# safijari/yag-slam

Hardware: AMD Instinct MI355X
Metric: pose hypotheses/sec (higher is better)
Workload: dtype u8

## Files before the change

### include/yagmatch.h

```cpp
#ifndef YAGMATCH_H
#define YAGMATCH_H

#include <stdint.h>

#ifdef __cplusplus
extern "C" {
#endif

#define YM_VERSION 1

enum {
    YM_OK = 0,
    YM_ERR_INVALID = -1,
    YM_ERR_NO_DEVICE = -2,
    YM_ERR_HIP = -3,
    YM_ERR_UNSUPPORTED = -4,
    YM_ERR_RANGE = -5,
    YM_ERR_BUSY = -6
};

enum { YM_SEM_KARTO = 0, YM_SEM_YAGPY = 1 };

typedef struct ym_config {
    double angle_variance_penalty;
// ... 215 lines not shown
int ym_graph_chi2(ym_graph *g, double *chi2);
int ym_graph_linearise(ym_graph *g, double *chi2, double *diag9 , double *grad3 );
int ym_graph_solve(ym_graph *g, int band , double lambda, double cg_tol, int max_cg_iters ,
                   double *delta3 , double *precond3 , int32_t *band_used,
                   int32_t *cg_iterations, double *residual, int32_t *flags);
typedef struct ym_opt_params { int32_t iters, exact, max_cg_iters, band ; double lambda0, cg_tol; } ym_opt_params;
typedef struct ym_opt_report { double chi2_initial, chi2_final, lambda_final; int32_t lm_steps, accepted, cg_iterations, band, status; } ym_opt_report;
int ym_graph_optimize(ym_graph *g, const ym_opt_params *p, ym_opt_report *out);

typedef struct ym_grid_info {
    int32_t width, height, pitch;
    int32_t origin_x, origin_y;
    int32_t storage_w, storage_h;
    int32_t roi_x, roi_y, roi_w, roi_h;
    double offset_x, offset_y;
} ym_grid_info;
int ym_debug_grid_info(ym_matcher *m, int item, ym_grid_info *info);
int ym_debug_grid(ym_matcher *m, int item, uint8_t *out, int64_t out_bytes);
int ym_debug_sums(ym_matcher *m, int item, int pass, uint32_t *out, int64_t out_count);
int ym_debug_map_sums(ym_matcher *m, int item, int pass, uint32_t *out, int64_t out_count);
int ym_debug_query_local(ym_matcher *m, int item, double *out_xy, int32_t cap, int32_t *n);
int ym_debug_cells(ym_matcher *m, int item, int32_t *out, int64_t out_count, int32_t *max_n);

int ym_debug_option(ym_matcher *m, int option, int value);

#define YM_DEBUG_COUNTERS 8
int ym_debug_counters(ym_matcher *m, int64_t *out, int32_t count);

int ym_debug_live_bytes(int64_t *device_bytes, int64_t *pinned_bytes);

int ym_debug_stamps(ym_matcher *m, int enable, uint64_t *out, int32_t count);

int ym_profile_enable(ym_matcher *m, int on);
int ym_profile_read(ym_matcher *m, int which, double *ms_total, int64_t *launches, int reset);
int ym_cache_stats(const ym_matcher *m, int64_t *hits, int64_t *misses);

#ifdef __cplusplus
}
#endif
#endif
```

### yag_slam_amd/_capi.py

```python
import ctypes as C
import os
import subprocess

_HERE = os.path.dirname(os.path.abspath(__file__))
LIB_PATH = os.environ.get("YM_LIB_PATH") or os.path.join(_HERE, "libyagmatch.so")

YM_OK = 0
SEM = {"karto": 0, "yagpy": 1}

EXPORTS = (
    "ym_version", "ym_build_id", "ym_device_count", "ym_last_error", "ym_create", "ym_destroy", "ym_get_config",
    "ym_set_stream", "ym_synchronize", "ym_scan_create", "ym_scans_create", "ym_scans_destroy", "ym_scan_set_pose", "ym_scans_set_poses", "ym_scan_get_pose",
    "ym_scan_size", "ym_scan_structure_trusted", "ym_scan_destroy", "ym_match", "ym_match_scans", "ym_map_sequence", "ym_process_scan", "ym_sequence_stats", "ym_async_slots",
    "ym_match_scans_async", "ym_wait", "ym_match_batch", "ym_batch_create", "ym_batch_destroy", "ym_batch_size",
    "ym_match_pairs", "ym_pairs_create",
    "ym_batch_run_async", "ym_batch_wait", "ym_debug_grid_info",
    "ym_debug_grid", "ym_debug_sums", "ym_debug_query_local", "ym_debug_cells", "ym_debug_option", "ym_debug_stamps", "ym_debug_live_bytes",
    "ym_profile_enable",
    "ym_profile_read", "ym_cache_stats", "ym_debug_counters",
    "ym_coarse_dims", "ym_match_slice_begin", "ym_match_slice_finish",
    "ym_occupancy_create", "ym_occupancy_create_counted", "ym_occupancy_get_info", "ym_occupancy_read", "ym_occupancy_read_counts",
    "ym_occupancy_destroy", "ym_image_despeckle", "ym_occupancy_create_clean", "ym_occupancy_get_despeckle_stats",
    "ym_map_from_occupancy", "ym_map_from_grid", "ym_map_size", "ym_map_read", "ym_map_destroy", "ym_match_map",
    "ym_match_map_many", "ym_map_track", "ym_debug_map_sums",
    "ym_raymap_create", "ym_raymap_trace", "ym_raymap_trace_each", "ym_raymap_destroy",
    "ym_locator_create", "ym_locator_get_info", "ym_locator_read_level", "ym_locator_locate", "ym_locator_destroy",
    "ym_segments_create", "ym_segments_label_range", "ym_segments_stats", "ym_segments_boundaries", "ym_segments_pairs",
    "ym_segments_destroy", "ym_map_free_space", "ym_segments_from_map", "ym_segments_labels",
    "ym_graph_create", "ym_graph_destroy", "ym_graph_add_nodes", "ym_graph_add_constraints", "ym_graph_size", "ym_graph_set_poses",
    "ym_graph_get_poses", "ym_graph_chi2", "ym_graph_linearise", "ym_graph_solve", "ym_graph_optimize",
)


class YmError(RuntimeError):
    def __init__(self, code, msg):
        super().__init__("libyagmatch error %d: %s" % (code, msg))
        self.code = code


class YmConfig(C.Structure):
# ... 165 lines not shown
    L.ym_match.argtypes = [vp, C.POINTER(YmScanDesc), C.POINTER(YmScanDesc), C.c_int, C.c_int, C.c_int,
                           C.POINTER(YmResult)]
    L.ym_match_scans.argtypes = [vp, vp, C.POINTER(vp), C.c_int, C.c_int, C.c_int, C.POINTER(YmResult)]
    L.ym_async_slots.argtypes = [vp]
    L.ym_match_scans_async.argtypes = [vp, vp, C.POINTER(vp), C.c_int, C.c_int, C.c_int, C.c_int]
    L.ym_wait.argtypes = [vp, C.c_int, C.POINTER(YmResult)]
    L.ym_match_batch.argtypes = [vp, vp, C.POINTER(vp), ip, C.c_int, C.c_int, C.c_int, C.POINTER(YmResult),
                                 C.POINTER(YmResult), ip]
    L.ym_batch_create.restype = vp
    L.ym_batch_create.argtypes = [vp, vp, C.POINTER(vp), ip, C.c_int]
    L.ym_pairs_create.restype = vp
    L.ym_pairs_create.argtypes = [vp, C.POINTER(vp), C.POINTER(vp), ip, C.c_int]
    L.ym_match_pairs.argtypes = [vp, C.POINTER(vp), C.POINTER(vp), ip, C.c_int, C.c_int, C.c_int, C.POINTER(YmResult)]
    L.ym_batch_destroy.argtypes = [vp]
    L.ym_batch_destroy.restype = None
    L.ym_batch_size.argtypes = [vp]
    L.ym_batch_run_async.argtypes = [vp, vp, C.c_int, C.c_int, C.c_int, C.c_int64, vp]
    L.ym_batch_wait.argtypes = [vp, C.c_int, C.POINTER(YmResult), C.POINTER(YmResult), ip]
    L.ym_debug_grid_info.argtypes = [vp, C.c_int, C.POINTER(YmGridInfo)]
    L.ym_debug_grid.argtypes = [vp, C.c_int, C.POINTER(C.c_uint8), C.c_int64]
    L.ym_debug_sums.argtypes = [vp, C.c_int, C.c_int, C.POINTER(C.c_uint32), C.c_int64]
    L.ym_debug_query_local.argtypes = [vp, C.c_int, dp, C.c_int32, ip]
    L.ym_debug_cells.argtypes = [vp, C.c_int, ip, C.c_int64, ip]
    L.ym_debug_option.argtypes = [vp, C.c_int, C.c_int]
    L.ym_debug_stamps.argtypes = [vp, C.c_int, C.POINTER(C.c_uint64), C.c_int32]
    L.ym_debug_live_bytes.argtypes = [C.POINTER(C.c_int64), C.POINTER(C.c_int64)]
    L.ym_profile_enable.argtypes = [vp, C.c_int]
    L.ym_profile_read.argtypes = [vp, C.c_int, dp, C.POINTER(C.c_int64), C.c_int]
    L.ym_cache_stats.argtypes = [vp, C.POINTER(C.c_int64), C.POINTER(C.c_int64)]
    L.ym_debug_counters.argtypes = [vp, C.POINTER(C.c_int64), C.c_int32]
    L.ym_coarse_dims.argtypes = [vp, ip]
    L.ym_scan_structure_trusted.argtypes = [vp, C.c_int]
    L.ym_process_scan.argtypes = [vp, vp, C.POINTER(vp), C.c_int, dp, dp, C.c_int, C.c_int, C.POINTER(YmResult)]
    L.ym_sequence_stats.argtypes = [vp, C.POINTER(C.c_int64), C.POINTER(C.c_int64), C.POINTER(C.c_int64)]
    L.ym_map_sequence.argtypes = [vp, C.POINTER(vp), dp, C.c_int, C.c_int, C.c_int, C.c_int, C.c_int, C.c_int, C.POINTER(YmResult), ip]
    L.ym_match_slice_begin.argtypes = [vp, vp, C.POINTER(vp), C.c_int, C.c_int, C.c_int, C.c_int, C.c_int, vp, vp]
    L.ym_match_slice_finish.argtypes = [vp, C.POINTER(YmResult)]
    L.ym_occupancy_create.restype = vp
    L.ym_occupancy_create.argtypes = [C.POINTER(vp), C.c_int, C.c_double, C.c_double]
    L.ym_occupancy_create_counted.restype = vp
    L.ym_occupancy_create_counted.argtypes = [C.POINTER(vp), C.c_int, C.c_double, C.c_double]
    L.ym_occupancy_get_info.argtypes = [vp, C.POINTER(YmOccupancyInfo)]
    L.ym_occupancy_read.argtypes = [vp, C.POINTER(C.c_uint8), C.c_int64]
    L.ym_occupancy_read_counts.argtypes = [vp, C.POINTER(C.c_uint32), C.POINTER(C.c_uint32), C.c_int64]
    L.ym_occupancy_destroy.argtypes = [vp]
    L.ym_occupancy_destroy.restype = None
# ... 93 lines not shown
```

### yag_slam_amd/csrc/ym_abi_debug.hpp

```cpp
int ym_debug_grid_info(ym_matcher *m, int item, ym_grid_info *info) {
    if (!m || !info) return set_err(YM_ERR_INVALID, "null argument");
    if (!m->last_valid || item < 0 || item >= m->last_B) return set_err(YM_ERR_INVALID, "no such item in the last call");
    const YmGeom &g = m->last_geom;
    info->width = g.win_w; info->height = g.win_w; info->pitch = g.pitch;
    info->origin_x = g.win_origin; info->origin_y = g.win_origin;
    info->storage_w = g.storage_w; info->storage_h = g.storage_w;
    info->roi_x = g.border; info->roi_y = g.border; info->roi_w = g.roi_w; info->roi_h = g.roi_w;
    YmItemState s;
    DEV_GUARD(m->device);
    HIP_TRY(hipStreamSynchronize(m->stream));
    HIP_TRY(hipMemcpy(&s, m->states.p + item, sizeof s, hipMemcpyDeviceToHost));
    info->offset_x = s.off_x; info->offset_y = s.off_y;
    return YM_OK;
}

int ym_debug_grid(ym_matcher *m, int item, uint8_t *out, int64_t out_bytes) {
    if (!m || !out) return set_err(YM_ERR_INVALID, "null argument");
    if (!m->last_valid || item < 0 || item >= m->last_B) return set_err(YM_ERR_INVALID, "no such item in the last call");
    const int64_t need = (int64_t)m->last_geom.pitch * m->last_geom.win_w;
    if (out_bytes < need) return set_err(YM_ERR_INVALID, "grid buffer too small: need %lld bytes", (long long)need);
    DEV_GUARD(m->device);
    HIP_TRY(hipStreamSynchronize(m->stream));
    HIP_TRY(hipMemcpy(out, m->grid.p + (size_t)item * m->last_grid_stride, (size_t)need, hipMemcpyDeviceToHost));
    return YM_OK;
// ... 18 lines not shown
    if (!m || !out_xy || !n) return set_err(YM_ERR_INVALID, "null argument");
    if (!m->last_valid || item < 0 || item >= m->last_B) return set_err(YM_ERR_INVALID, "no such item in the last call");
    YmItemState s;
    DEV_GUARD(m->device);
    HIP_TRY(hipStreamSynchronize(m->stream));
    HIP_TRY(hipMemcpy(&s, m->states.p + item, sizeof s, hipMemcpyDeviceToHost));
    *n = s.nq;
    if (cap < s.nq) return set_err(YM_ERR_INVALID, "buffer too small: need %d points", s.nq);
    if (s.nq > 0)
        HIP_TRY(hipMemcpy(out_xy, s.ql, sizeof(double2) * s.nq, hipMemcpyDeviceToHost));
    return YM_OK;
}

int ym_debug_cells(ym_matcher *m, int item, int32_t *out, int64_t out_count, int32_t *max_n) {
    if (!m || !max_n) return set_err(YM_ERR_INVALID, "null argument");
    if (!m->last_valid || item < 0 || item >= m->last_B) return set_err(YM_ERR_INVALID, "no such item in the last call");
    *max_n = m->last_max_n;
    const size_t per = (size_t)m->last_max_base * m->last_max_n;
    if (!out) return YM_OK;
    if ((size_t)out_count < per * 2) return set_err(YM_ERR_INVALID, "buffer too small: need %zu ints", per * 2);
    DEV_GUARD(m->device);
    HIP_TRY(hipStreamSynchronize(m->stream));
    HIP_TRY(hipMemcpy(out, m->cells.p + (size_t)item * per, sizeof(int2) * per, hipMemcpyDeviceToHost));
    return YM_OK;
}

int ym_debug_option(ym_matcher *m, int option, int value) {
    if (m) { m->cache_gen++; m->list_key_valid = false; }
    if (!m) return set_err(YM_ERR_INVALID, "null matcher");
    if (option == 0) return set_err(YM_ERR_INVALID, "debug option 0 (an experimental correlate form) no longer exists");
    else if (option == 2) m->full_raster = value;
    else if (option == 3) m->corr_u = value;
    else if (option == 4) m->corr_pad_lds = value;
    else if (option == 5) m->corr_chunks = value;
    else if (option == 6) m->finish_form = value;
    else if (option == 9) m->corr_cw = value;
    else if (option == 10) m->select_global = value;
    else if (option == 41) m->select_split_max = value;
    else if (option == 11) m->finish_threads = value;
    else if (option == 12) m->keep_sums = value;
    else if (option == 13) m->corr_dedup = value;
    else if (option == 14) m->corr_region = value;
    else if (option == 15) m->corr_region_na = m->corr_region_nw = value;
    else if (option == 23) m->poll_completion = value != 0;
    else if (option == 24) m->use_scan_structure = value != 0;
    else if (option == 25) m->chain_margin = value;
// ... 148 lines not shown
```

### yag_slam_amd/csrc/ym_host_call.hpp

```cpp
int launch_call_body(ym_matcher *m, Slot &slot) {
    static const bool debug_host = getenv("YM_DEBUG_HOST") != nullptr;
    timespec t_[8];
    auto mark = [&](int i) { if (debug_host) clock_gettime(CLOCK_MONOTONIC, &t_[i]); };
    mark(7);
    DEV_GUARD(m->device);
    CallPlan P;
    int rc;
    mark(0);
    m->last_corr_form = -1;
    if ((rc = plan_sizes(m, slot, P))) return rc;
    mark(1);
    Call &pc = slot.call;
    const bool replay = pc.batch_uid != 0 && pc.plan_clean && pc.plan_gen == m->cache_gen && pc.pose_epoch == g_pose_epoch.load(std::memory_order_relaxed);
    if (!replay && (rc = plan_cache(m, slot, P))) return rc;
    mark(2);
    if ((rc = plan_jobs(m, slot, P, replay))) return rc;
    mark(3);
    if ((rc = plan_descriptor(m, slot, P, replay))) return rc;
    if (pc.batch_uid != 0 && !replay) {
        bool clean = !m->cache_off;
        for (const CallScan &cs : pc.scans) clean = clean && !cs.stale && !cs.qstale;
        pc.plan_clean = clean;
        pc.plan_gen = m->cache_gen;
    }
    mark(4);
    hipStream_t st = m->stream;
    hipEvent_t ev_call = nullptr;
    if ((rc = prof_begin(m, 2, &ev_call))) return rc;
    if ((rc = plan_raster(m, slot, P))) return rc;
    mark(5);

    timespec e_[8];
// ... 316 lines not shown
```

### yag_slam_amd/csrc/ym_host_enqueue.hpp

```cpp
void enqueue_prepare(ym_matcher *m, const CallPlan &P) {
    ym::PrepareArgs a;
    a.scans = P.d_scans; a.items = P.d_items; a.g = P.g; a.lat = P.lc; a.states = m->states.p; a.qlocal = m->qlocal.p;
    a.cells = m->cells.p; a.bbox = m->bbox.p; a.ctrig = m->ctrig.p; a.hypcell = m->hypcell.p; a.probs = P.probs;
    a.max_n = P.max_n; a.max_base = P.max_base; a.nt_stride = P.nt_stride; a.dim_stride = P.dim_stride; a.stamps = P.stamps;
    a.use_inline = P.inline_desc ? 1 : 0;
    a.pad0 = 0;
    std::memset(&a.inl, 0, sizeof a.inl);
    if (a.use_inline) {
        a.inl.item = P.hi[0];
        for (int i = 0; i < P.nscans; i++) a.inl.scans[i] = P.hs[i];
    }
    a.qnp = m->qnp.p; a.jobs = P.d_jobs; a.job_slot = P.d_job_slot;
    a.fault = nullptr; a.step = 0; a.pad1 = 0;
    for (int k = 0; k < 4; k++) a.cell_box[k] = P.cell_box[k];
    if (P.chain_step) { a.fault = m->seq_fault.p; a.step = P.chain_step; }
    a.tile_max_zero = P.use_tile_list ? m->tile_max.p : nullptr;
    const size_t lds = YM_PREP_LDS_BYTES(P.max_n);
    if (P.split_prepare) {
        if (P.n_jobs > 0) hipLaunchKernelGGL(ym::points_kernel, dim3(P.n_jobs), dim3(YM_POINTS_THREADS), lds, m->stream, a);
        hipLaunchKernelGGL(ym::cells_kernel, dim3(P.max_base + 1, P.B), dim3(256), 0, m->stream, a);
    } else {
        if (P.B == 1 && m->prepare_threads != 512)
            hipLaunchKernelGGL(ym::prepare_kernel<1024>, dim3(P.max_base + 2, P.B), dim3(1024), lds, m->stream, a);
        else
// ... 162 lines not shown
    if (P.rg2) { r.rg_h = P.rg2_h; r.rg_cls = YM_RG_PITCH * (P.rg2_h + 26); r.rg_zero = 4 * r.rg_cls; }
    r.pad2 = ((1 << 21) + r.rg_h - 1) / r.rg_h;
    r.rg_w = 0; r.rg_pitch = YM_RG_PITCH; r.nregions = P.rg_nregions; r.pad3 = 0;
    r.walk = m->rg_walk.p; r.nitems = P.B; r.rsplit = P.rg_rsplit; r.pad4 = 0;
    r.lnw = P.rg_lnw; r.lparts = P.rg_lparts; r.entries_pstride = P.rg_entries_pstride;
    r.gpx = std::max(1, std::min((2 * std::max(m->n_cus, 8) / 8) / std::max(1, P.rg_parts), (P.B + 7) / 8));
    return r;
}

int enqueue_region_lists(ym_matcher *m, const CallPlan &P, hipStream_t st) {
    const ym::RegionArgs r = region_args(m, P);
#ifdef YM_EXPERIMENTAL
    if (P.rg_lparts == 1 && P.rg_lnw == P.lc.nt && (P.rg_ws || P.rg2 || P.rg_item || P.rg_pool)) {
        const size_t bin_lds = YM_BIN_LDS_BYTES(P.rg_nbins, P.rg_entries_stride, P.rg_nregions * P.rg_parts);
        if (bin_lds > m->bin_lds_limit) {
            HIP_TRY(hipFuncSetAttribute(reinterpret_cast<const void *>(ym::bin_whole_kernel<false>), hipFuncAttributeMaxDynamicSharedMemorySize, (int)bin_lds));
            m->bin_lds_limit = bin_lds;
        }
        hipLaunchKernelGGL(ym::bin_whole_kernel<false>, dim3(P.n_qslots), dim3(YM_BIN_THREADS), bin_lds, st, r);
        if (P.rg_ws) hipLaunchKernelGGL(ym::region_walk_kernel, dim3(P.rg_parts, P.n_qslots), dim3(64), 0, st, r);
        return YM_OK;
    }
#endif
    const size_t bin_lds = YM_BINP_LDS_BYTES(P.rg_nbins, P.rg_entries_pstride, P.rg_nregions);
    if (bin_lds > m->binp_lds_limit) {
#define YM_BINP_ATTR(Y, M) HIP_TRY(hipFuncSetAttribute(reinterpret_cast<const void *>(ym::bin_kernel<Y, M>), hipFuncAttributeMaxDynamicSharedMemorySize, (int)bin_lds))
        YM_BINP_ATTR(false, 18); YM_BINP_ATTR(false, 32); YM_BINP_ATTR(false, 64); YM_BINP_ATTR(true, 18); YM_BINP_ATTR(true, 32); YM_BINP_ATTR(true, 64);
#undef YM_BINP_ATTR
        m->binp_lds_limit = bin_lds;
    }
    const int per_thread = (P.rg_lnw * P.max_n + YM_BINP_THREADS - 1) / YM_BINP_THREADS;
    const dim3 bgrid(P.rg_lparts, P.n_qslots);
#define YM_BINP_LAUNCH(Y, M) hipLaunchKernelGGL((ym::bin_kernel<Y, M>), bgrid, dim3(YM_BINP_THREADS), bin_lds, st, r)
    if (P.yag) { if (per_thread <= 18) YM_BINP_LAUNCH(true, 18); else if (per_thread <= 32) YM_BINP_LAUNCH(true, 32); else YM_BINP_LAUNCH(true, 64); }
    else { if (per_thread <= 18) YM_BINP_LAUNCH(false, 18); else if (per_thread <= 32) YM_BINP_LAUNCH(false, 32); else YM_BINP_LAUNCH(false, 64); }
#undef YM_BINP_LAUNCH
    return YM_OK;
}

int enqueue_region_lists_aside(ym_matcher *m, CallPlan &P) {
    if (!m->side_stream) {
        HIP_TRY(hipStreamCreateWithFlags(&m->side_stream, hipStreamNonBlocking));
        pool_register_stream(m->device, m->side_stream, true);
        HIP_TRY(hipEventCreateWithFlags(&m->ev_fork, hipEventDisableTiming));
        HIP_TRY(hipEventCreateWithFlags(&m->ev_join, hipEventDisableTiming));
    }
    HIP_TRY(hipEventRecord(m->ev_fork, m->stream));
    return YM_OK;
}
int enqueue_region_lists_joined(ym_matcher *m, CallPlan &P) {
    HIP_TRY(hipStreamWaitEvent(m->side_stream, m->ev_fork, 0));
    int rc = enqueue_region_lists(m, P, m->side_stream);
    if (rc) return rc;
    HIP_TRY(hipEventRecord(m->ev_join, m->side_stream));
    P.lists_on_side_stream = true;
    return YM_OK;
}

// ... 211 lines not shown
```

### yag_slam_amd/csrc/ym_host_matcher.hpp

```cpp
struct ym_map {
    int device;
    int width, height;
    DevBuf<double> d_cgrid;
    DevBuf<uint8_t> d_g8;
};

struct ym_occupancy {
    int device;
    ym_occupancy_info info;
    std::vector<uint8_t> image;
    std::vector<uint32_t> counts;
    bool cleaned = false;
    ym_despeckle_stats clean_stats{};
};

struct ym_batch {
    std::vector<const ym_scan *> queries;
    std::vector<int32_t> item_query;
    std::vector<const ym_scan *> scans;
    std::vector<int32_t> offsets;
    mutable std::vector<int> cache_hints;
    mutable std::vector<int> query_hints;
    uint64_t uid = 0;
};
// ... 126 lines not shown
    int corr_pad_lds = 0;
    int corr_cw = 0;
    int corr_dedup = 0;
    int corr_region = 0;
    int corr_region_na = 0;
    int corr_region_parts = 0;
    int corr_region_cap = 0;
    int corr_region_lds = 0;
    int raster_gx = 0;
    int raster_hits_per_tile = 0;
    int keep_sums = 0;
    int finish_threads = 0;
    int select_global = 0;
    int select_split_max = 8;
    DevBuf<double> tmp_ranges;
    PinnedBuf tmp_ranges_host;
    Slot slots[kAsyncSlots + 1];
    YmGeom last_geom;
    YmLattice last_lat[2];
    int last_B = 0, last_max_n = 0, last_max_base = 0, last_nt_stride = 0, last_dim_stride = 0;
    size_t last_grid_stride = 0, last_sums_stride[2] = {0, 0};
    size_t sums_pass_offset[2] = {0, 0};
    bool last_valid = false;
    bool profiling = false;
    ProfEvents prof[3];
};
```

### yag_slam_amd/csrc/ym_k_region.hpp

```cpp
#pragma once

namespace ym {

#ifndef YM_RG_PROF
#define YM_RG_PROF 0
#endif
#if YM_RG_PROF
#if YM_RG_PROF == 2
#define YM_RG_PH(i) do { if ((i) == 7 || (i) == 8 || (i) == 1 || (i) == 2 || (i) == 5) { const uint32_t t_ = (uint32_t)__builtin_amdgcn_s_memtime(); \
    if ((i) != 5) ph[(i) == 7 ? 0 : (i) == 8 ? 1 : (i) == 1 ? 2 : 3] += t_ - pt; pt = t_; } } while (0)
#else
#define YM_RG_PH(i) do { const uint32_t t_ = (uint32_t)__builtin_amdgcn_s_memtime(); if ((i) >= 2 && (i) <= 5) ph[(i) - 2] += t_ - pt; pt = t_; } while (0)
#endif
#else
#define YM_RG_PH(i) do { } while (0)
#endif

#ifndef YM_RG_ABLATE
#define YM_RG_ABLATE 0
#endif
#ifndef YM_RG_PRIO
#define YM_RG_PRIO 0
#endif
#define YM_RG_W 64
// ... 79 lines not shown
        const unsigned rx = xc / (unsigned)a.rg_w, ry = yc / (unsigned)a.rg_h;
        if ((int)rx >= a.nrx || (int)ry >= a.nry) return false;
        region = (int)((ry * (unsigned)a.nrx + rx) * 4u + cls);
        bin = region * a.lat.nt + k;
        er = yc - ry * (unsigned)a.rg_h;
        ex = xc - rx * (unsigned)a.rg_w;
        entry = er * (unsigned)a.rg_pitch + ex;
        return true;
    }
#endif
    if (yc >= 4096u) return false;
    const unsigned rx = xc / (unsigned)YM_RG_W, ry = __umul24(yc, (unsigned)a.pad2) >> 21;
    if ((int)rx >= a.nrx || (int)ry >= a.nry) return false;
    region = (int)(__umul24(ry, (unsigned)a.nrx) + rx);
    bin = (int)__umul24((unsigned)region, (unsigned)(bin_nw < 0 ? a.lat.nt : bin_nw)) + k;
    er = yc - __umul24(ry, (unsigned)a.rg_h);
    ex = xc - rx * YM_RG_W;
    entry = __umul24(cls, (unsigned)a.rg_cls) + __umul24(er, (unsigned)YM_RG_PITCH) + ex;
    return true;
}

#define YM_BINP_THREADS 512
#define YM_BINP_LDS_BYTES(nbins, entries, nboxes) ((size_t)(YM_BINP_THREADS / 64 + 16 + YM_RG_MAX_BINS / 32 + 1) * 4 + (size_t)(nbins) * 8 + ((size_t)(entries) * 2 + 15) / 16 * 16 + (size_t)(nboxes) * 16)
template <bool YAG, int MAXP>
__global__ __launch_bounds__(YM_BINP_THREADS, MAXP <= 18 ? 4 : 2) void bin_kernel(RegionArgs a) {
    constexpr int NT = YM_BINP_THREADS;
    extern __shared__ __attribute__((aligned(16))) unsigned char bin_smem[];
    int *wave_tot = reinterpret_cast<int *>(bin_smem);
    int *angle_tot = wave_tot + NT / 64;
    unsigned *region_bits = reinterpret_cast<unsigned *>(angle_tot + 16);
    int *regions_used = reinterpret_cast<int *>(region_bits + YM_RG_MAX_BINS / 32);
    unsigned (*cnt)[2] = reinterpret_cast<unsigned (*)[2]>(regions_used + 1);
    unsigned short *ent = reinterpret_cast<unsigned short *>(cnt + a.nbins);
    const int nboxes = a.nregions;
    unsigned (*box)[4] = reinterpret_cast<unsigned (*)[4]>(bin_smem + ((reinterpret_cast<unsigned char *>(ent + a.entries_pstride) - bin_smem) + 15) / 16 * 16);
    const int part = blockIdx.x, qs = blockIdx.y, b = a.qrep[qs], tid = threadIdx.x, lane = tid & 63;
    const YmItemState &st = a.states[b];
    const int nw = a.lnw, k_lo = part * nw, nk = min(a.lat.nt, k_lo + nw) - k_lo;
    const int nq = st.nq;
    const int total = nq * nk;
    const int32_t *cx = a.hypcell + (size_t)b * 2 * a.dim_stride;
    const int cx0 = cx[0], cy0 = cx[a.dim_stride];
    const double off_x = st.off_x, off_y = st.off_y;
    const double2 *ql = reinterpret_cast<const double2 *>(st.ql);
    const double2 *trig = a.ctrig + (size_t)b * a.nt_stride + k_lo;
    int32_t *starts = a.starts + (size_t)qs * a.starts_stride + (size_t)part * (a.nbins + 1);
    int32_t *flag = a.starts + (size_t)qs * a.starts_stride + (size_t)a.lparts * (a.nbins + 1) + part;
    const int pos0 = part * (int)a.entries_pstride;
    double2 *qls = reinterpret_cast<double2 *>(bin_smem + ((reinterpret_cast<unsigned char *>(ent) - bin_smem) + 15) / 16 * 16);
    const bool ql_in_lds = (size_t)(nq + nk) * sizeof(double2) + 16 <= (size_t)a.entries_pstride * 2;
    double2 *trigs = qls + nq;
    if (ql_in_lds) {
        for (int i = tid; i < nq; i += NT) qls[i] = ql[i];
        if (tid < nk) trigs[tid] = trig[tid];
    }
    for (int i = tid; i < a.nbins * 2; i += NT) (&cnt[0][0])[i] = 0u;
    if (tid < 16) angle_tot[tid] = 0;
    if (tid < YM_RG_MAX_BINS / 32) region_bits[tid] = 0u;
    if (tid == 0) *regions_used = 0;
    for (int i = tid; i < nboxes; i += NT) { box[i][0] = 255u; box[i][1] = 0u; box[i][2] = 255u; box[i][3] = 0u; }
    __syncthreads();
    unsigned key[MAXP];
    unsigned rank_hi[(MAXP + 3) / 4];
#pragma unroll
    for (int q = 0; q < (MAXP + 3) / 4; q++) rank_hi[q] = 0u;
    const int per_thread = (total + NT - 1) / NT;
    const int p0 = tid * per_thread;
    int k = p0 / max(nq, 1), i = p0 - k * nq;
    int cur = -1;
    unsigned r0 = 255u, r1 = 0u, x0 = 255u, x1 = 0u;
    auto send_box = [&]() {
        if (cur >= 0) {
            unsigned *bx = box[cur];
            atomicMin(&bx[0], r0); atomicMax(&bx[1], r1); atomicMin(&bx[2], x0); atomicMax(&bx[3], x1);
        }
    };
    bool overflow = per_thread > MAXP;
    auto pass1 = [&](auto point_of, auto trig_of) {
#pragma unroll
        for (int q = 0; q < MAXP; q++) {
            const int pp = p0 + q;
            key[q] = 0xffffffffu;
            if (q < per_thread && pp < total) {
                const double2 cs = trig_of(k);
                const double2 pt = point_of(i);
                int bin, region; unsigned e, er, ex;
                const int2 lc = YAG ? lookup_cell_sem(a.g, pt, cs.x, cs.y, off_x, off_y, st.ylat[0], st.ylat[1]) : lookup_cell(pt, cs.x, cs.y, off_x, off_y, a.g.scale);
                if (region_entry(a, lc, cx0, cy0, k, bin, e, region, er, ex, nw)) {
                    const unsigned rank = (atomicAdd(&cnt[bin][(e >> 1) & 1u], 1u << (16 * (e & 1u))) >> (16 * (e & 1u))) & 0xffffu;
                    key[q] = (rank & 7u) << 29 | (unsigned)bin << 16 | e;
                    rank_hi[q >> 2] |= ((rank >> 3) & 0xffu) << (8 * (q & 3));
                    if (region != cur) { send_box(); cur = region; r0 = r1 = er; x0 = x1 = ex; }
                    else { r0 = min(r0, er); r1 = max(r1, er); x0 = min(x0, ex); x1 = max(x1, ex); }
                }
            }
            if (++i >= nq) { i = 0; k++; }
        }
    };
    if (ql_in_lds) pass1([&](int i_) { return qls[i_]; }, [&](int k_) { return trigs[k_]; });
    else pass1([&](int i_) { return ql[i_]; }, [&](int k_) { return trig[k_]; });
    send_box();
    __syncthreads();
    {
        uint32_t *rb = a.rbox + (size_t)qs * a.rbox_stride;
        for (int r = tid; r < nboxes; r += NT) rb[(size_t)r * a.lparts + part] = box[r][0] | box[r][1] << 8 | box[r][2] << 16 | box[r][3] << 24;
    }
    const int per = (a.nbins + NT - 1) / NT;
    const int first = tid * per;
    int padded_total;
    {
        int local = 0;
        for (int j = 0; j < per; j++)
            if (first + j < a.nbins) {
                const unsigned c01 = cnt[first + j][0], c23 = cnt[first + j][1];
                const int c[4] = {(int)(c01 & 0xffffu), (int)(c01 >> 16), (int)(c23 & 0xffffu), (int)(c23 >> 16)};
                const int padded = (((c[0] + 1) & ~1) + ((c[1] + 1) & ~1) + ((c[2] + 1) & ~1) + ((c[3] + 1) & ~1) + 3) & ~3;
                local += padded;
                if (padded) {
                    atomicAdd(&angle_tot[(first + j) % nw], padded);
                    const int R = (first + j) / nw;
                    atomicOr(&region_bits[R >> 5], 1u << (R & 31));
                }
            }
// ... 26 lines not shown
                unsigned fill[4];
                for (int r = 0; r < 4; r++) {
                    fill[r] = (unsigned)pos;
                    if (fits && (c[r] & 1)) ent[pos + c[r]] = (unsigned short)(a.rg_zero + r);
                    pos += (c[r] + 1) & ~1;
                }
                if (fits && ((pos - run) & 3)) { ent[pos] = (unsigned short)a.rg_zero; ent[pos + 1] = (unsigned short)a.rg_zero; }
                pos = run + ((pos - run + 3) & ~3);
                cnt[first + j][0] = fill[0] | fill[1] << 16;
                cnt[first + j][1] = fill[2] | fill[3] << 16;
                run = pos;
            }
        if (tid == 0) {
            starts[a.nbins] = pos0 + all;
            *flag = fits ? all : -1;
            if (a.stamps && qs == 0 && part == 0) a.stamps[26] = (unsigned long long)all;
        }
        if (!fits) return;
    }
    __syncthreads();
#pragma unroll
    for (int q = 0; q < MAXP; q++) {
        if (key[q] == 0xffffffffu) continue;
        const unsigned bin = (key[q] >> 16) & 0x1fffu, e = key[q] & 0xffffu;
        const unsigned rank = key[q] >> 29 | ((rank_hi[q >> 2] >> (8 * (q & 3))) & 0xffu) << 3;
        const unsigned f = cnt[bin][(e >> 1) & 1u];
        ent[((e & 1u) ? f >> 16 : f & 0xffffu) + rank] = (unsigned short)e;
    }
    __syncthreads();
    uint32_t *out = reinterpret_cast<uint32_t *>(a.entries + (size_t)qs * a.entries_stride + pos0);
    const uint32_t *src = reinterpret_cast<const uint32_t *>(ent);
    for (int i2 = tid; i2 < (padded_total + 1) / 2; i2 += NT) out[i2] = src[i2];
}

typedef unsigned int rg_u32x2 __attribute__((ext_vector_type(2)));
__device__ __forceinline__ void rg_perm_pair(const rg_u32x2 &pa, const rg_u32x2 &qa, const rg_u32x2 &pb, const rg_u32x2 &qb, uint32_t rr,
                                             uint32_t (&e)[4], uint32_t (&o)[4]) {
    const uint32_t s0 = pa.x + pb.x, s1 = pa.y + pb.y, s2 = qa.x + qb.x, s3 = qa.y + qb.y;
    const uint32_t selE = rr * 0x00010001u + 0x0c020c00u, selO = selE + 0x00010001u;
    e[0] = __builtin_amdgcn_perm(s1, s0, selE); o[0] = __builtin_amdgcn_perm(s1, s0, selO);
    e[1] = __builtin_amdgcn_perm(s2, s1, selE); o[1] = __builtin_amdgcn_perm(s2, s1, selO);
    e[2] = __builtin_amdgcn_perm(s3, s2, selE); o[2] = __builtin_amdgcn_perm(s3, s2, selO);
    e[3] = __builtin_amdgcn_perm(0u, s3, selE);
    o[3] = 0u;
}
__device__ __forceinline__ void rg_gather4(uint32_t (&acc)[8], uint32_t lane_off, uint2 ee ) {
    const uint32_t ad0 = lane_off + (ee.x & 0xffffu), ad1 = lane_off + (ee.x >> 16), ad2 = lane_off + (ee.y & 0xffffu), ad3 = lane_off + (ee.y >> 16);
#if YM_RG_ABLATE & 1
    acc[0] += ad0 ^ ad1 ^ ad2 ^ ad3;
    return;
#endif
    rg_u32x2 p0, q0, p1, q1, p2, q2, p3, q3;
    asm volatile("ds_read2_b32 %0, %8 offset1:1\n\tds_read2_b32 %1, %8 offset0:2 offset1:3\n\t"
                 "ds_read2_b32 %2, %9 offset1:1\n\tds_read2_b32 %3, %9 offset0:2 offset1:3\n\t"
                 "ds_read2_b32 %4, %10 offset1:1\n\tds_read2_b32 %5, %10 offset0:2 offset1:3\n\t"
                 "ds_read2_b32 %6, %11 offset1:1\n\tds_read2_b32 %7, %11 offset0:2 offset1:3\n\t"
// ... 327 lines not shown
```

### yag_slam_amd/scan_matching.py

```python
import ctypes as C
import os
import struct
from collections import namedtuple

import numpy as np

from . import _capi
from .config import default_config, default_config_loop, make_config
from .models import LocalizedRangeScan
from .transform import Transform

ScanMatcherResult = namedtuple('ScanMatcherResult', ['response', 'covariance', 'best_pose', 'meta'])


def _pose_of(scan):
    p = scan.corrected_pose
    return float(p.x), float(p.y), float(p.euler[-1])


def _desc_of(scan, keep):
    d = _capi.YmScanDesc()
    r = np.ascontiguousarray(scan.ranges, dtype=np.float64)
    keep.append(r)
    d.ranges = r.ctypes.data_as(C.POINTER(C.c_double))
# ... 474 lines not shown
        _capi.check(self._lib.ym_debug_sums(self._m, item, pass_, buf.ctypes.data_as(C.POINTER(C.c_uint32)), buf.size))
        return buf

    def debug_map_sums(self, pass_=0, item=0, dims=None):
        nx, ny, nt = dims
        buf = np.zeros((nt, ny, nx), dtype=np.uint32)
        _capi.check(self._lib.ym_debug_map_sums(self._m, int(item), int(pass_), buf.ctypes.data_as(C.POINTER(C.c_uint32)), buf.size))
        return buf

    def debug_query_local(self, item=0, cap=8192):
        buf = np.zeros((cap, 2))
        n = C.c_int32()
        _capi.check(self._lib.ym_debug_query_local(self._m, item, buf.ctypes.data_as(C.POINTER(C.c_double)), cap,
                                                   C.byref(n)))
        return buf[:n.value].copy()

    def debug_cells(self, item=0, cap=1 << 16):
        buf = np.zeros((cap, 2), dtype=np.int32)
        max_n = C.c_int32()
        _capi.check(self._lib.ym_debug_cells(self._m, item, buf.ctypes.data_as(C.POINTER(C.c_int32)), buf.size,
                                             C.byref(max_n)))
        return buf.reshape(-1, 2), max_n.value

    def debug_option(self, option, value):
        _capi.check(self._lib.ym_debug_option(self._m, int(option), int(value)))

    def debug_stamps(self, enable=True):
        buf = (C.c_uint64 * 32)()
        _capi.check(self._lib.ym_debug_stamps(self._m, int(bool(enable)), buf, 32))
        return list(buf)

    def cache_stats(self):
        h, ms = C.c_int64(0), C.c_int64(0)
        _capi.check(self._lib.ym_cache_stats(self._m, C.byref(h), C.byref(ms)))
        return int(h.value), int(ms.value)

    def debug_counters(self):
        buf = (C.c_int64 * 8)()
        _capi.check(self._lib.ym_debug_counters(self._m, buf, 8))
        return dict(yag_fast_items=int(buf[0]), yag_fallback_items=int(buf[1]), yag_pairs_checked=int(buf[2]),
                    yag_pairs_failed=int(buf[3]), list_cache_hits=int(buf[4]), map_kernel_items=int(buf[6]), map_fallback_items=int(buf[7]),
                    last_correlate={-1: None, 0: "correlate_kernel", 1: "correlate_region_kernel", 2: "gather_kernel"}[int(buf[5])])

    def profile(self, on=True):
        _capi.check(self._lib.ym_profile_enable(self._m, int(bool(on))))

# ... 223 lines not shown
```

Before: 13.45 billion.

## Restructure bin kernel: angle-major thread mapping, LDS/memory variants, packed ranks

The region bin kernel now gives each thread a fixed angle and a contiguous run of query points, so trig is loaded once per thread and the per-point div/mod index stepping disappears. It is split into two template variants, one staging query points in LDS and one reading them from global memory, chosen on the host, which removes the runtime branch. Bin/element index math is replaced with mul24 arithmetic, ranks are packed three 11-bit values per register, and box min/max use packed 16-bit ops. Launch bounds allow more blocks for the small non-YAG case. A debug API for dumping the region lists is also added. The new thread mapping can be uneven when nq does not divide well across threads per angle, and raising the occupancy hint may put pressure on registers.

```diff
diff --git a/include/yagmatch.h b/include/yagmatch.h
--- a/include/yagmatch.h
+++ b/include/yagmatch.h
@@ -261,6 +261,9 @@
 int ym_debug_query_local(ym_matcher *m, int item, double *out_xy, int32_t cap, int32_t *n);
 int ym_debug_cells(ym_matcher *m, int item, int32_t *out, int64_t out_count, int32_t *max_n);
 
+int ym_debug_region_lists(ym_matcher *m, int qslot, int item, int32_t *info, double *geom, int32_t geom_count, uint16_t *entries,
+                          int64_t entries_count, int32_t *starts, int64_t starts_count, uint32_t *rbox, int64_t rbox_count);
+
 int ym_debug_option(ym_matcher *m, int option, int value);
 
 #define YM_DEBUG_COUNTERS 8
diff --git a/yag_slam_amd/_capi.py b/yag_slam_amd/_capi.py
--- a/yag_slam_amd/_capi.py
+++ b/yag_slam_amd/_capi.py
@@ -15,7 +15,7 @@
     "ym_match_scans_async", "ym_wait", "ym_match_batch", "ym_batch_create", "ym_batch_destroy", "ym_batch_size",
     "ym_match_pairs", "ym_pairs_create",
     "ym_batch_run_async", "ym_batch_wait", "ym_debug_grid_info",
-    "ym_debug_grid", "ym_debug_sums", "ym_debug_query_local", "ym_debug_cells", "ym_debug_option", "ym_debug_stamps", "ym_debug_live_bytes",
+    "ym_debug_grid", "ym_debug_sums", "ym_debug_query_local", "ym_debug_cells", "ym_debug_region_lists", "ym_debug_option", "ym_debug_stamps", "ym_debug_live_bytes",
     "ym_profile_enable",
     "ym_profile_read", "ym_cache_stats", "ym_debug_counters",
     "ym_coarse_dims", "ym_match_slice_begin", "ym_match_slice_finish",
@@ -227,6 +227,8 @@
     L.ym_debug_sums.argtypes = [vp, C.c_int, C.c_int, C.POINTER(C.c_uint32), C.c_int64]
     L.ym_debug_query_local.argtypes = [vp, C.c_int, dp, C.c_int32, ip]
     L.ym_debug_cells.argtypes = [vp, C.c_int, ip, C.c_int64, ip]
+    L.ym_debug_region_lists.argtypes = [vp, C.c_int, C.c_int, ip, dp, C.c_int32, C.POINTER(C.c_uint16), C.c_int64, ip, C.c_int64,
+                                        C.POINTER(C.c_uint32), C.c_int64]
     L.ym_debug_option.argtypes = [vp, C.c_int, C.c_int]
     L.ym_debug_stamps.argtypes = [vp, C.c_int, C.POINTER(C.c_uint64), C.c_int32]
     L.ym_debug_live_bytes.argtypes = [C.POINTER(C.c_int64), C.POINTER(C.c_int64)]
diff --git a/yag_slam_amd/csrc/ym_abi_debug.hpp b/yag_slam_amd/csrc/ym_abi_debug.hpp
--- a/yag_slam_amd/csrc/ym_abi_debug.hpp
+++ b/yag_slam_amd/csrc/ym_abi_debug.hpp
@@ -64,6 +64,45 @@
     DEV_GUARD(m->device);
     HIP_TRY(hipStreamSynchronize(m->stream));
     HIP_TRY(hipMemcpy(out, m->cells.p + (size_t)item * per, sizeof(int2) * per, hipMemcpyDeviceToHost));
+    return YM_OK;
+}
+
+int ym_debug_region_lists(ym_matcher *m, int qslot, int item, int32_t *info, double *geom, int32_t geom_count, uint16_t *entries, int64_t entries_count,
+                          int32_t *starts, int64_t starts_count, uint32_t *rbox, int64_t rbox_count) {
+    if (!m || !info) return set_err(YM_ERR_INVALID, "null argument");
+    if (!m->last_valid || item < 0 || item >= m->last_B) return set_err(YM_ERR_INVALID, "no such item in the last call");
+    if (qslot < 0 || qslot >= m->last_lists_qslots) return set_err(YM_ERR_INVALID, "the last call built no pair lists for query slot %d", qslot);
+    const ym::RegionArgs &a = m->last_lists;
+    const int nt = a.lat.nt;
+    const size_t n_entries = (size_t)a.lparts * a.entries_pstride, n_starts = (size_t)a.lparts * (a.nbins + 1) + a.lparts, n_rbox = (size_t)a.nregions * a.lparts;
+    DEV_GUARD(m->device);
+    HIP_TRY(hipStreamSynchronize(m->stream));
+    if (m->side_stream) HIP_TRY(hipStreamSynchronize(m->side_stream));
+    YmItemState s;
+    int32_t c0[2];
+    HIP_TRY(hipMemcpy(&s, m->states.p + item, sizeof s, hipMemcpyDeviceToHost));
+    HIP_TRY(hipMemcpy(&c0[0], a.hypcell + (size_t)item * 2 * a.dim_stride, sizeof(int32_t), hipMemcpyDeviceToHost));
+    HIP_TRY(hipMemcpy(&c0[1], a.hypcell + (size_t)item * 2 * a.dim_stride + a.dim_stride, sizeof(int32_t), hipMemcpyDeviceToHost));
+    const int32_t v[16] = {a.lparts, a.lnw, a.nbins, a.nregions, a.nrx, a.nry, a.rg_h, a.rg_cls, a.rg_zero, (int32_t)a.entries_pstride, nt, s.nq, c0[0], c0[1],
+                           YM_RG_W, YM_RG_PITCH};
+    std::memcpy(info, v, sizeof v);
+    if (geom) {
+        if (geom_count < 3 + 2 * nt) return set_err(YM_ERR_INVALID, "geometry buffer too small: need %d doubles", 3 + 2 * nt);
+        geom[0] = s.off_x; geom[1] = s.off_y; geom[2] = a.g.scale;
+        HIP_TRY(hipMemcpy(geom + 3, a.ctrig + (size_t)item * a.nt_stride, sizeof(double2) * nt, hipMemcpyDeviceToHost));
+    }
+    if (entries) {
+        if (entries_count < 0 || (size_t)entries_count < n_entries) return set_err(YM_ERR_INVALID, "entry buffer too small: need %zu", n_entries);
+        HIP_TRY(hipMemcpy(entries, a.entries + (size_t)qslot * a.entries_stride, n_entries * sizeof(uint16_t), hipMemcpyDeviceToHost));
+    }
+    if (starts) {
+        if (starts_count < 0 || (size_t)starts_count < n_starts) return set_err(YM_ERR_INVALID, "starts buffer too small: need %zu", n_starts);
+        HIP_TRY(hipMemcpy(starts, a.starts + (size_t)qslot * a.starts_stride, n_starts * sizeof(int32_t), hipMemcpyDeviceToHost));
+    }
+    if (rbox) {
+        if (rbox_count < 0 || (size_t)rbox_count < n_rbox) return set_err(YM_ERR_INVALID, "box buffer too small: need %zu", n_rbox);
+        HIP_TRY(hipMemcpy(rbox, a.rbox + (size_t)qslot * a.rbox_stride, n_rbox * sizeof(uint32_t), hipMemcpyDeviceToHost));
+    }
     return YM_OK;
 }
 
diff --git a/yag_slam_amd/csrc/ym_host_call.hpp b/yag_slam_amd/csrc/ym_host_call.hpp
--- a/yag_slam_amd/csrc/ym_host_call.hpp
+++ b/yag_slam_amd/csrc/ym_host_call.hpp
@@ -8,6 +8,7 @@
     int rc;
     mark(0);
     m->last_corr_form = -1;
+    m->last_lists_qslots = 0;
     if ((rc = plan_sizes(m, slot, P))) return rc;
     mark(1);
     Call &pc = slot.call;
diff --git a/yag_slam_amd/csrc/ym_host_enqueue.hpp b/yag_slam_amd/csrc/ym_host_enqueue.hpp
--- a/yag_slam_amd/csrc/ym_host_enqueue.hpp
+++ b/yag_slam_amd/csrc/ym_host_enqueue.hpp
@@ -208,18 +208,23 @@
         return YM_OK;
     }
 #endif
+    m->last_lists = r; m->last_lists_qslots = P.n_qslots;
     const size_t bin_lds = YM_BINP_LDS_BYTES(P.rg_nbins, P.rg_entries_pstride, P.rg_nregions);
     if (bin_lds > m->binp_lds_limit) {
-#define YM_BINP_ATTR(Y, M) HIP_TRY(hipFuncSetAttribute(reinterpret_cast<const void *>(ym::bin_kernel<Y, M>), hipFuncAttributeMaxDynamicSharedMemorySize, (int)bin_lds))
+#define YM_BINP_ATTR(Y, M) HIP_TRY(hipFuncSetAttribute(reinterpret_cast<const void *>(ym::bin_kernel<Y, M>), hipFuncAttributeMaxDynamicSharedMemorySize, (int)bin_lds)); \
+                           HIP_TRY(hipFuncSetAttribute(reinterpret_cast<const void *>(ym::bin_mem_kernel<Y, M>), hipFuncAttributeMaxDynamicSharedMemorySize, (int)bin_lds))
         YM_BINP_ATTR(false, 18); YM_BINP_ATTR(false, 32); YM_BINP_ATTR(false, 64); YM_BINP_ATTR(true, 18); YM_BINP_ATTR(true, 32); YM_BINP_ATTR(true, 64);
 #undef YM_BINP_ATTR
         m->binp_lds_limit = bin_lds;
     }
-    const int per_thread = (P.rg_lnw * P.max_n + YM_BINP_THREADS - 1) / YM_BINP_THREADS;
+    const int per_thread = YM_BINP_PER_THREAD(P.max_n, std::max(1, P.rg_lnw));
+    const int maxp = per_thread <= 18 ? 18 : per_thread <= 32 ? 32 : 64;
+    const bool qlds = YM_BINP_QL_FITS(P.max_n, maxp, P.rg_entries_pstride);
     const dim3 bgrid(P.rg_lparts, P.n_qslots);
-#define YM_BINP_LAUNCH(Y, M) hipLaunchKernelGGL((ym::bin_kernel<Y, M>), bgrid, dim3(YM_BINP_THREADS), bin_lds, st, r)
-    if (P.yag) { if (per_thread <= 18) YM_BINP_LAUNCH(true, 18); else if (per_thread <= 32) YM_BINP_LAUNCH(true, 32); else YM_BINP_LAUNCH(true, 64); }
-    else { if (per_thread <= 18) YM_BINP_LAUNCH(false, 18); else if (per_thread <= 32) YM_BINP_LAUNCH(false, 32); else YM_BINP_LAUNCH(false, 64); }
+#define YM_BINP_LAUNCH(Y, M) do { if (qlds) hipLaunchKernelGGL((ym::bin_kernel<Y, M>), bgrid, dim3(YM_BINP_THREADS), bin_lds, st, r); \
+                                  else hipLaunchKernelGGL((ym::bin_mem_kernel<Y, M>), bgrid, dim3(YM_BINP_THREADS), bin_lds, st, r); } while (0)
+    if (P.yag) { if (maxp == 18) YM_BINP_LAUNCH(true, 18); else if (maxp == 32) YM_BINP_LAUNCH(true, 32); else YM_BINP_LAUNCH(true, 64); }
+    else { if (maxp == 18) YM_BINP_LAUNCH(false, 18); else if (maxp == 32) YM_BINP_LAUNCH(false, 32); else YM_BINP_LAUNCH(false, 64); }
 #undef YM_BINP_LAUNCH
     return YM_OK;
 }
diff --git a/yag_slam_amd/csrc/ym_host_matcher.hpp b/yag_slam_amd/csrc/ym_host_matcher.hpp
--- a/yag_slam_amd/csrc/ym_host_matcher.hpp
+++ b/yag_slam_amd/csrc/ym_host_matcher.hpp
@@ -172,6 +172,8 @@
     size_t last_grid_stride = 0, last_sums_stride[2] = {0, 0};
     size_t sums_pass_offset[2] = {0, 0};
     bool last_valid = false;
+    ym::RegionArgs last_lists;
+    int last_lists_qslots = 0;
     bool profiling = false;
     ProfEvents prof[3];
 };
diff --git a/yag_slam_amd/csrc/ym_k_region.hpp b/yag_slam_amd/csrc/ym_k_region.hpp
--- a/yag_slam_amd/csrc/ym_k_region.hpp
+++ b/yag_slam_amd/csrc/ym_k_region.hpp
@@ -125,8 +125,22 @@
 
 #define YM_BINP_THREADS 512
 #define YM_BINP_LDS_BYTES(nbins, entries, nboxes) ((size_t)(YM_BINP_THREADS / 64 + 16 + YM_RG_MAX_BINS / 32 + 1) * 4 + (size_t)(nbins) * 8 + ((size_t)(entries) * 2 + 15) / 16 * 16 + (size_t)(nboxes) * 16)
-template <bool YAG, int MAXP>
-__global__ __launch_bounds__(YM_BINP_THREADS, MAXP <= 18 ? 4 : 2) void bin_kernel(RegionArgs a) {
+#define YM_BINP_QL_FITS(n, maxp, entries) (((size_t)(n) + (size_t)(maxp)) * 16 + 16 <= (size_t)(entries) * 2)
+#define YM_BINP_PER_THREAD(n, angles) (((n) + YM_BINP_THREADS / (angles) - 1) / (YM_BINP_THREADS / (angles)))
+typedef unsigned short binp_u16x2 __attribute__((ext_vector_type(2)));
+__device__ __forceinline__ int binp_round_int(double v) { return (int)copysign(fabs(v) + 0.5, v); }
+__device__ __forceinline__ int2 binp_lookup_cell(double2 p, double cosine, double sine, double off_x, double off_y, double scale) {
+    const double ox = cosine * p.x - sine * p.y;
+    const double oy = sine * p.x + cosine * p.y;
+    return make_int2(binp_round_int(((ox + off_x) - off_x) * scale), binp_round_int(((oy + off_y) - off_y) * scale));
+}
+__device__ __forceinline__ unsigned binp_mul24(unsigned a, unsigned b) {
+    unsigned r;
+    asm("v_mul_u32_u24 %0, %1, %2" : "=v"(r) : "s"(b), "v"(a));
+    return r;
+}
+template <bool YAG, int MAXP, bool QLDS>
+__device__ __forceinline__ void bin_block(const RegionArgs &a) {
     constexpr int NT = YM_BINP_THREADS;
     extern __shared__ __attribute__((aligned(16))) unsigned char bin_smem[];
     int *wave_tot = reinterpret_cast<int *>(bin_smem);
@@ -140,8 +154,8 @@
     const int part = blockIdx.x, qs = blockIdx.y, b = a.qrep[qs], tid = threadIdx.x, lane = tid & 63;
     const YmItemState &st = a.states[b];
     const int nw = a.lnw, k_lo = part * nw, nk = min(a.lat.nt, k_lo + nw) - k_lo;
-    const int nq = st.nq;
-    const int total = nq * nk;
+    const bool ql_room = !QLDS || YM_BINP_QL_FITS(st.nq, MAXP, a.entries_pstride);
+    const int nq = ql_room ? st.nq : 0;
     const int32_t *cx = a.hypcell + (size_t)b * 2 * a.dim_stride;
     const int cx0 = cx[0], cy0 = cx[a.dim_stride];
     const double off_x = st.off_x, off_y = st.off_y;
@@ -150,13 +164,9 @@
     int32_t *starts = a.starts + (size_t)qs * a.starts_stride + (size_t)part * (a.nbins + 1);
     int32_t *flag = a.starts + (size_t)qs * a.starts_stride + (size_t)a.lparts * (a.nbins + 1) + part;
     const int pos0 = part * (int)a.entries_pstride;
-    double2 *qls = reinterpret_cast<double2 *>(bin_smem + ((reinterpret_cast<unsigned char *>(ent) - bin_smem) + 15) / 16 * 16);
-    const bool ql_in_lds = (size_t)(nq + nk) * sizeof(double2) + 16 <= (size_t)a.entries_pstride * 2;
-    double2 *trigs = qls + nq;
-    if (ql_in_lds) {
-        for (int i = tid; i < nq; i += NT) qls[i] = ql[i];
-        if (tid < nk) trigs[tid] = trig[tid];
-    }
+    const double2 *qls = reinterpret_cast<const double2 *>(bin_smem + ((reinterpret_cast<unsigned char *>(ent) - bin_smem) + 15) / 16 * 16);
+    if (QLDS)
+        for (int i = tid; i < nq; i += NT) const_cast<double2 *>(qls)[i] = ql[i];
     for (int i = tid; i < a.nbins * 2; i += NT) (&cnt[0][0])[i] = 0u;
     if (tid < 16) angle_tot[tid] = 0;
     if (tid < YM_RG_MAX_BINS / 32) region_bits[tid] = 0u;
@@ -164,44 +174,48 @@
     for (int i = tid; i < nboxes; i += NT) { box[i][0] = 255u; box[i][1] = 0u; box[i][2] = 255u; box[i][3] = 0u; }
     __syncthreads();
     unsigned key[MAXP];
-    unsigned rank_hi[(MAXP + 3) / 4];
-#pragma unroll
-    for (int q = 0; q < (MAXP + 3) / 4; q++) rank_hi[q] = 0u;
-    const int per_thread = (total + NT - 1) / NT;
-    const int p0 = tid * per_thread;
-    int k = p0 / max(nq, 1), i = p0 - k * nq;
-    int cur = -1;
-    unsigned r0 = 255u, r1 = 0u, x0 = 255u, x1 = 0u;
+    unsigned rank3[(MAXP + 2) / 3];
+#pragma unroll
+    for (int q = 0; q < (MAXP + 2) / 3; q++) rank3[q] = 0u;
+    const int tpa = NT / max(nk, 1), per_thread = (nq + tpa - 1) / tpa;
+    const int k = max(min(tid / tpa, nk - 1), 0);
+    const int nvalid = tid < nk * tpa ? min(nq - (tid - k * tpa) * per_thread, per_thread) : 0;
+    const int i0 = min((tid - k * tpa) * per_thread, nq);
+    const bool overflow = per_thread > MAXP || !ql_room;
+    const double2 cs = trig[k];
+    const unsigned pad2 = (unsigned)a.pad2, rg_h = (unsigned)a.rg_h, nrx = (unsigned)a.nrx, rg_cls = (unsigned)a.rg_cls;
+    const unsigned x_end = nrx * (2u * YM_RG_W), y_end = 2u * min(4096u, (unsigned)a.nry * rg_h);
+    const unsigned nw8 = (unsigned)nw * 8u, k8 = (unsigned)k * 8u;
+    unsigned cur = 0u, bmin = 0xffffffffu, bmax = 0u;
     auto send_box = [&]() {
-        if (cur >= 0) {
-            unsigned *bx = box[cur];
-            atomicMin(&bx[0], r0); atomicMax(&bx[1], r1); atomicMin(&bx[2], x0); atomicMax(&bx[3], x1);
-        }
+        unsigned *bx = box[cur];
+        atomicMin(&bx[0], bmin & 0xffffu); atomicMax(&bx[1], bmax & 0xffffu); atomicMin(&bx[2], bmin >> 16); atomicMax(&bx[3], bmax >> 16);
     };
-    bool overflow = per_thread > MAXP;
-    auto pass1 = [&](auto point_of, auto trig_of) {
-#pragma unroll
-        for (int q = 0; q < MAXP; q++) {
-            const int pp = p0 + q;
-            key[q] = 0xffffffffu;
-            if (q < per_thread && pp < total) {
-                const double2 cs = trig_of(k);
-                const double2 pt = point_of(i);
-                int bin, region; unsigned e, er, ex;
-                const int2 lc = YAG ? lookup_cell_sem(a.g, pt, cs.x, cs.y, off_x, off_y, st.ylat[0], st.ylat[1]) : lookup_cell(pt, cs.x, cs.y, off_x, off_y, a.g.scale);
-                if (region_entry(a, lc, cx0, cy0, k, bin, e, region, er, ex, nw)) {
-                    const unsigned rank = (atomicAdd(&cnt[bin][(e >> 1) & 1u], 1u << (16 * (e & 1u))) >> (16 * (e & 1u))) & 0xffffu;
-                    key[q] = (rank & 7u) << 29 | (unsigned)bin << 16 | e;
-                    rank_hi[q >> 2] |= ((rank >> 3) & 0xffu) << (8 * (q & 3));
-                    if (region != cur) { send_box(); cur = region; r0 = r1 = er; x0 = x1 = ex; }
-                    else { r0 = min(r0, er); r1 = max(r1, er); x0 = min(x0, ex); x1 = max(x1, ex); }
-                }
-            }
-            if (++i >= nq) { i = 0; k++; }
-        }
-    };
-    if (ql_in_lds) pass1([&](int i_) { return qls[i_]; }, [&](int k_) { return trigs[k_]; });
-    else pass1([&](int i_) { return ql[i_]; }, [&](int k_) { return trig[k_]; });
+#pragma unroll
+    for (int q = 0; q < MAXP; q++) {
+        double2 pt;
+        if (QLDS) pt = qls[i0 + q];
+        else pt = q < nvalid ? ql[i0 + q] : make_double2(0.0, 0.0);
+        const int2 lc = YAG ? lookup_cell_sem(a.g, pt, cs.x, cs.y, off_x, off_y, st.ylat[0], st.ylat[1]) : binp_lookup_cell(pt, cs.x, cs.y, off_x, off_y, a.g.scale);
+        const unsigned X = (unsigned)(cx0 + lc.x), Y = (unsigned)(cy0 + lc.y);
+        key[q] = 0xffffffffu;
+        if (q < nvalid && X < x_end && Y < y_end) {
+            const unsigned yc = Y >> 1, ry = binp_mul24(yc, pad2) >> 21, er = yc - __umul24(ry, rg_h), ex = (X >> 1) & (YM_RG_W - 1);
+            const unsigned region = __umul24(ry, nrx) + (X >> 7);
+            const unsigned bin8 = __umul24(region, nw8) + k8;
+            const unsigned e = __umul24((X & 1u) | ((Y & 1u) << 1), rg_cls) + __umul24(er, (unsigned)YM_RG_PITCH) + ex;
+            const unsigned sh = (X << 3) & 16u;
+            const unsigned rank = __builtin_amdgcn_ubfe(atomicAdd(reinterpret_cast<unsigned *>(reinterpret_cast<unsigned char *>(cnt) + (bin8 | (X & 4u))), 1u << sh), sh, 11u);
+            key[q] = bin8 << 13 | e;
+            if (q % 3) rank3[q / 3] |= rank << (11 * (q % 3));
+            else rank3[q / 3] = rank;
+            const unsigned erx = er | ex << 16;
+            if (q == 0) { cur = region; bmin = bmax = erx; }
+            else if (region != cur) { send_box(); cur = region; bmin = bmax = erx; }
+            bmin = __builtin_bit_cast(unsigned, __builtin_elementwise_min(__builtin_bit_cast(binp_u16x2, bmin), __builtin_bit_cast(binp_u16x2, erx)));
+            bmax = __builtin_bit_cast(unsigned, __builtin_elementwise_max(__builtin_bit_cast(binp_u16x2, bmax), __builtin_bit_cast(binp_u16x2, erx)));
+        }
+    }
     send_box();
     __syncthreads();
     {
@@ -274,8 +288,8 @@
 #pragma unroll
     for (int q = 0; q < MAXP; q++) {
         if (key[q] == 0xffffffffu) continue;
-        const unsigned bin = (key[q] >> 16) & 0x1fffu, e = key[q] & 0xffffu;
-        const unsigned rank = key[q] >> 29 | ((rank_hi[q >> 2] >> (8 * (q & 3))) & 0xffu) << 3;
+        const unsigned bin = key[q] >> 16, e = key[q] & 0xffffu;
+        const unsigned rank = (rank3[q / 3] >> (11 * (q % 3))) & 0x7ffu;
         const unsigned f = cnt[bin][(e >> 1) & 1u];
         ent[((e & 1u) ? f >> 16 : f & 0xffffu) + rank] = (unsigned short)e;
     }
@@ -284,6 +298,10 @@
     const uint32_t *src = reinterpret_cast<const uint32_t *>(ent);
     for (int i2 = tid; i2 < (padded_total + 1) / 2; i2 += NT) out[i2] = src[i2];
 }
+template <bool YAG, int MAXP>
+__global__ __launch_bounds__(YM_BINP_THREADS, MAXP > 18 ? 2 : YAG ? 4 : 8) void bin_kernel(RegionArgs a) { bin_block<YAG, MAXP, true>(a); }
+template <bool YAG, int MAXP>
+__global__ __launch_bounds__(YM_BINP_THREADS, MAXP > 18 ? 2 : YAG ? 4 : 8) void bin_mem_kernel(RegionArgs a) { bin_block<YAG, MAXP, false>(a); }
 
 typedef unsigned int rg_u32x2 __attribute__((ext_vector_type(2)));
 __device__ __forceinline__ void rg_perm_pair(const rg_u32x2 &pa, const rg_u32x2 &qa, const rg_u32x2 &pb, const rg_u32x2 &qb, uint32_t rr,
diff --git a/yag_slam_amd/scan_matching.py b/yag_slam_amd/scan_matching.py
--- a/yag_slam_amd/scan_matching.py
+++ b/yag_slam_amd/scan_matching.py
@@ -520,6 +520,24 @@
                                              C.byref(max_n)))
         return buf.reshape(-1, 2), max_n.value
 
+    def debug_region_lists(self, qslot=0, item=0):
+        info = (C.c_int32 * 16)()
+        none16, none32u = C.POINTER(C.c_uint16)(), C.POINTER(C.c_uint32)()
+        _capi.check(self._lib.ym_debug_region_lists(self._m, int(qslot), int(item), info, None, 0, none16, 0, None, 0, none32u, 0))
+        keys = ("parts", "lnw", "nbins", "nregions", "nrx", "nry", "rg_h", "rg_cls", "rg_zero", "room", "nt", "nq", "cx0", "cy0", "rg_w", "rg_pitch")
+        d = dict(zip(keys, (int(v) for v in info)))
+        geom = np.zeros(3 + 2 * d["nt"])
+        entries = np.zeros((d["parts"], d["room"]), dtype=np.uint16)
+        starts = np.zeros(d["parts"] * (d["nbins"] + 1) + d["parts"], dtype=np.int32)
+        rbox = np.zeros((d["nregions"], d["parts"]), dtype=np.uint32)
+        _capi.check(self._lib.ym_debug_region_lists(self._m, int(qslot), int(item), info, geom.ctypes.data_as(C.POINTER(C.c_double)), geom.size,
+                                                    entries.ctypes.data_as(C.POINTER(C.c_uint16)), entries.size,
+                                                    starts.ctypes.data_as(C.POINTER(C.c_int32)), starts.size,
+                                                    rbox.ctypes.data_as(C.POINTER(C.c_uint32)), rbox.size))
+        d.update(off_x=geom[0], off_y=geom[1], scale=geom[2], trig=geom[3:].reshape(-1, 2), entries=entries,
+                 starts=starts[:d["parts"] * (d["nbins"] + 1)].reshape(d["parts"], d["nbins"] + 1), flags=starts[d["parts"] * (d["nbins"] + 1):], rbox=rbox)
+        return d
+
     def debug_option(self, option, value):
         _capi.check(self._lib.ym_debug_option(self._m, int(option), int(value)))
 
```

Result: no change. 13.53 billion (median of 6 runs) (+0.6%).
